# c-zhou/oatk

Measured on AMD Instinct MI355X. Metric: HiFi Gbases/s through syncasm (syncmer+syncerr) at k=1001 s=31, higher is better.
Workload: dtype u64

## Files before the change

oatk_amd/csrc/api.hip:

```cpp
#include <hip/hip_runtime.h>
#include <rocprim/device/device_radix_sort.hpp>
#include <rocprim/device/device_scan.hpp>
#include <rocprim/device/device_transform.hpp>
#include <stdio.h>
#include <stdlib.h>
#include <string.h>
#include <time.h>
#include <execinfo.h>
#include <sys/mman.h>
#include <condition_variable>
#include <mutex>
#include <string>
#include <thread>
#include <utility>
#include <vector>

#include "../../include/oatk_hip.h"
#include "common.hpp"
#include "scan_hpc.hpp"
#include "scan_syncmer.hpp"
#include "scan_syncmer_fast.hpp"
#include "kmer_hash.hpp"
#include "count.hpp"

// ... 734 lines not shown
{
    uint64_t i = (uint64_t) blockIdx.x * blockDim.x + threadIdx.x;
    if (i < n) iota[first + i] = (uint32_t) (first + i);
}

static void scan_reset_downstream(oatk_hip_ctx *ctx)
{
    ctx->scanned = ctx->counted = false;
    ctx->slots_packed = false;
    if (ctx->ec) ctx->ec->done = ctx->ec->marked = ctx->ec->graph_resident = ctx->ec->global = false;
    if (ctx->cons) ctx->cons->done = false;
    if (ctx->ag) ctx->ag->done = false;
    if (ctx->ovl) ctx->ovl->done = false;
    if (ctx->ra) ctx->ra->done = false;
    if (ctx->multi) ctx->multi->merged = ctx->multi->ec_done = false;
}

int oatk_hip_device(oatk_hip_ctx *ctx) { return ctx? ctx->device : -1; }

int oatk_hip_d2d(oatk_hip_ctx *ctx, void *d_dst, const void *d_src, uint64_t bytes)
{
    if (!ctx) return OATK_E_NODEV;
    if (bytes == 0) return OATK_OK;
    CK(hipSetDevice(ctx->device));
    CK(hipMemcpyAsync(d_dst, d_src, bytes, hipMemcpyDeviceToDevice, ctx->stream));
    CK(hipStreamSynchronize(ctx->stream));
    return OATK_OK;
}

int oatk_hip_scan_begin(oatk_hip_ctx *ctx, uint64_t sid0, int k, int s)
{
    if (!ctx) return OATK_E_NODEV;
    CK(hipSetDevice(ctx->device));
    if (!(s > 0 && s < 32 && k > s) || k > oatk_hip_max_k()) { ctx->err = "k/s out of range for the device scan"; return OATK_E_ARG; }
    scan_reset_downstream(ctx);
    ctx->d_seq = nullptr, ctx->d_off = nullptr, ctx->d_len = nullptr;
    ctx->n_reads = 0, ctx->seq_bytes = 0, ctx->sid0 = sid0, ctx->K = k, ctx->S = s;
    ctx->retries = 0, ctx->collisions = 0;
    ctx->n_occ = ctx->tot_nn = ctx->tot_lrl = ctx->n_scm_total = 0;
    ctx->nn_sorted_in_2 = ctx->lrl_sorted_in_2 = false;
    ctx->scanned = true;
    return OATK_OK;
}

#define KEEP(buf, bytes, used)                                                                     \
    do {                                                                                           \
        if (!ctx->buf.grow_keep((bytes), (used), ctx->stream)) {                                   \
            ctx->err = "hipMalloc failed for " #buf " (append)";                                   \
            return OATK_E_NOMEM;                                                                   \
        }                                                                                          \
    } while (0)

static int append_ensure(oatk_hip_ctx *ctx, uint64_t nr, uint64_t sb, uint64_t occ, uint64_t nn, uint64_t lrl)
{
    const uint64_t n0 = ctx->n_reads, b0 = ctx->seq_bytes, o0 = ctx->n_occ;
    KEEP(in_off, (nr + 1) * 8, n0 * 8);
    KEEP(hoco_l, nr * 4 + 4, n0 * 4); KEEP(n_scm, nr * 4 + 4, n0 * 4); KEEP(n_nn, nr * 4 + 4, n0 * 4); KEEP(n_lrl, nr * 4 + 4, n0 * 4);
    KEEP(ho_rl, sb + 64, b0);
    KEEP(hoco_s, sb / 4 + 128 + 16 + ctx->import_reserve, b0 / 4 + 64);
    KEEP(scm_off, (nr + 1) * 8, (n0 + 1) * 8);
    KEEP(pos_hash, occ * 8 + 8, o0 * 8); KEEP(pos_lo, occ * 8 + 8, o0 * 8); KEEP(pos_smer, occ * 8 + 8, o0 * 8); KEEP(pos_mpos, occ * 4 + 4, o0 * 4);
    KEEP(key_hash, occ * 8 + 8, o0 * 8); KEEP(iota, occ * 4 + 4, o0 * 4);
    KEEP(nn_key, nn * 8 + 8, ctx->tot_nn * 8); KEEP(lrl_key, lrl * 8 + 8, ctx->tot_lrl * 8); KEEP(lrl_val, lrl * 4 + 4, ctx->tot_lrl * 4);
    return OATK_OK;
}

int oatk_hip_scan_reserve(oatk_hip_ctx *ctx, uint64_t seq_bytes, uint64_t n_reads, uint64_t n_occ)
{
    if (!ctx) return OATK_E_NODEV;
    CK(hipSetDevice(ctx->device));
    if (!ctx->scanned || ctx->d_seq) { ctx->err = "oatk_hip_scan_reserve: call oatk_hip_scan_begin first"; return OATK_E_STATE; }
    seq_bytes = (seq_bytes + 63) & ~63ULL;
    if (pool_of_current_device()) {
        const uint64_t sb = ctx->seq_bytes + seq_bytes;
        if (!ctx->ho_rl.reserve(sb + 64, ctx->seq_bytes, ctx->stream) || !ctx->hoco_s.reserve(sb / 4 + 128 + 16 + ctx->import_reserve, ctx->seq_bytes / 4 + 64, ctx->stream)) {
            ctx->err = "oatk_hip_scan_reserve: no address range for the batch";
            return OATK_E_NOMEM;
        }
        return OATK_OK;
    }
    return append_ensure(ctx, ctx->n_reads + n_reads, ctx->seq_bytes + seq_bytes, ctx->n_occ + n_occ, ctx->tot_nn, ctx->tot_lrl);
}

int oatk_hip_scan_append(oatk_hip_ctx *ctx, oatk_hip_ctx *src)
{
    if (!ctx || !src) return OATK_E_NODEV;
    CK(hipSetDevice(ctx->device));
    if (ctx == src || ctx->device != src->device) { ctx->err = "oatk_hip_scan_append: the piece must be another handle on the same device"; return OATK_E_ARG; }
    if (!ctx->scanned || ctx->d_seq) { ctx->err = "oatk_hip_scan_append: call oatk_hip_scan_begin first"; return OATK_E_STATE; }
    if (!src->scanned) { ctx->err = "oatk_hip_scan_append: the piece holds no scan"; return OATK_E_STATE; }
    const uint64_t n0 = ctx->n_reads, n1 = src->n_reads, b0 = ctx->seq_bytes, b1 = src->seq_bytes, o0 = ctx->n_occ, o1 = src->n_occ;
    if (n1 == 0) return OATK_OK;
    if (src->K != ctx->K || src->S != ctx->S) { ctx->err = "oatk_hip_scan_append: the piece was scanned with another k / s"; return OATK_E_ARG; }
    if (src->sid0 != ctx->sid0 + n0) { ctx->err = "oatk_hip_scan_append: the piece's first read id must continue the batch"; return OATK_E_ARG; }
    if (n0 + n1 >= 0xFFFFFFFFULL || o0 + o1 > 0xFFFFFFF0ULL) { ctx->err = "oatk_hip_scan_append: batch too large"; return OATK_E_ARG; }
    scan_reset_downstream(ctx);
    ctx->scanned = true;
    { int rc = append_ensure(ctx, n0 + n1, b0 + b1, o0 + o1, ctx->tot_nn + src->tot_nn, ctx->tot_lrl + src->tot_lrl); if (rc) return rc; }
    if (hipStreamSynchronize(src->stream) != hipSuccess) { ctx->err = "oatk_hip_scan_append: the piece's stream failed"; return OATK_E_NODEV; }
    hipStream_t st = ctx->stream;
    auto blocks = [](uint64_t n) { return dim3((unsigned) ((n + 255) / 256 > 0? (n + 255) / 256 : 1)); };
    auto d2d = [&](void *dst, const void *from, size_t bytes) { return bytes? hipMemcpyAsync(dst, from, bytes, hipMemcpyDeviceToDevice, st) : hipSuccess; };
    CK(d2d(ctx->ho_rl.as<uint8_t>() + b0, src->ho_rl.p, b1));
    CK(d2d(ctx->hoco_s.as<uint8_t>() + b0 / 4, src->hoco_s.p, b1 / 4 + 64));
    CK(d2d(ctx->hoco_l.as<uint32_t>() + n0, src->hoco_l.p, n1 * 4)); CK(d2d(ctx->n_scm.as<uint32_t>() + n0, src->n_scm.p, n1 * 4));
    CK(d2d(ctx->n_nn.as<uint32_t>() + n0, src->n_nn.p, n1 * 4)); CK(d2d(ctx->n_lrl.as<uint32_t>() + n0, src->n_lrl.p, n1 * 4));
    hipLaunchKernelGGL(append_rebase_kernel, blocks(n1), dim3(256), 0, st, src->d_off, ctx->in_off.as<uint64_t>() + n0, n1, b0);
    hipLaunchKernelGGL(append_rebase_kernel, blocks(n1 + 1), dim3(256), 0, st, src->scm_off.as<uint64_t>(), ctx->scm_off.as<uint64_t>() + n0, n1 + 1, o0);
    if (o1) {
        CK(d2d(ctx->pos_hash.as<uint64_t>() + o0, src->pos_hash.p, o1 * 8)); CK(d2d(ctx->pos_lo.as<uint64_t>() + o0, src->pos_lo.p, o1 * 8));
        CK(d2d(ctx->pos_smer.as<uint64_t>() + o0, src->pos_smer.p, o1 * 8)); CK(d2d(ctx->pos_mpos.as<uint32_t>() + o0, src->pos_mpos.p, o1 * 4));
        CK(d2d(ctx->key_hash.as<uint64_t>() + o0, src->key_hash.p, o1 * 8));
        hipLaunchKernelGGL(append_iota_kernel, blocks(o1), dim3(256), 0, st, ctx->iota.as<uint32_t>(), o0, o1);
    }
    CK(d2d(ctx->nn_key.as<uint64_t>() + ctx->tot_nn, src->nn_sorted_in_2? src->nn_key2.p : src->nn_key.p, src->tot_nn * 8));
    CK(d2d(ctx->lrl_key.as<uint64_t>() + ctx->tot_lrl, src->lrl_sorted_in_2? src->lrl_key2.p : src->lrl_key.p, src->tot_lrl * 8));
    CK(d2d(ctx->lrl_val.as<uint32_t>() + ctx->tot_lrl, src->lrl_sorted_in_2? src->lrl_val2.p : src->lrl_val.p, src->tot_lrl * 4));
    CK(hipGetLastError());
    CK(hipStreamSynchronize(st));
    ctx->d_off = ctx->in_off.as<uint64_t>();
    ctx->n_reads = n0 + n1, ctx->seq_bytes = b0 + b1, ctx->n_occ = o0 + o1;
    ctx->tot_nn += src->tot_nn, ctx->tot_lrl += src->tot_lrl;
    ctx->retries += src->retries;
    return OATK_OK;
}

int oatk_hip_scan_host(oatk_hip_ctx *ctx, const uint8_t *h_seq, const uint64_t *h_off, const uint32_t *h_len,
                       uint64_t n_reads, uint64_t seq_bytes, uint64_t sid0, int k, int s)
{
    if (!ctx) return OATK_E_NODEV;
    CK(hipSetDevice(ctx->device));
    ENSURE(in_seq, seq_bytes + 64); ENSURE(in_off, (n_reads + 1) * 8); ENSURE(in_len, (n_reads + 1) * 4);
    if (seq_bytes) CK(hipMemcpyAsync(ctx->in_seq.p, h_seq, seq_bytes, hipMemcpyHostToDevice, ctx->stream));
    if (n_reads) {
        CK(hipMemcpyAsync(ctx->in_off.p, h_off, n_reads * 8, hipMemcpyHostToDevice, ctx->stream));
        CK(hipMemcpyAsync(ctx->in_len.p, h_len, n_reads * 4, hipMemcpyHostToDevice, ctx->stream));
    }
    return oatk_hip_scan(ctx, ctx->in_seq.as<uint8_t>(), ctx->in_off.as<uint64_t>(), ctx->in_len.as<uint32_t>(), n_reads, seq_bytes, sid0, k, s);
}

int oatk_hip_count(oatk_hip_ctx *ctx)
{
    using namespace oatk;
    if (!ctx) return OATK_E_NODEV;
    if (!ctx->scanned) { ctx->err = "count before scan"; return OATK_E_STATE; }
    CK(hipSetDevice(ctx->device));
    ctx->counted = false;
    ctx->n_scm_total = 0;
    if (ctx->multi) ctx->multi->merged = ctx->multi->ec_done = false;
    const uint64_t n = ctx->n_occ;
    if (n == 0) { ctx->counted = true; return OATK_OK; }
    const unsigned nb = (unsigned) ((n + 255) / 256);

    ENSURE(key_sorted, n * 8); ENSURE(perm, n * 4); ENSURE(head, n * 4); ENSURE(head_idx, n * 4); ENSURE(newclus, n * 4); ENSURE(kloc, n * 8);
    if (ctx->seq_bytes >> 4 >= 0xFFFFFFFFULL) { ctx->err = "batch too large for 32-bit hoco word indices (64 GB of bases)"; return OATK_E_ARG; }
    ENSURE(clus_id, n * 4); ENSURE(bad_head, n * 4); ENSURE(tag, n * 4); ENSURE(tmp_perm, n * 4); ENSURE(flags, 64);
    ENSURE(pos_kid, n * 8); ENSURE(scm_occ, n * 8);
    CK(hipMemsetAsync(ctx->flags.p, 0, 64, ctx->stream));

    bool full_sort = getenv("OATK_DEBUG_FULL_SORT") != nullptr || n < (1ull << 22);
sort_again:
    t_begin(ctx, OATK_T_COUNT_SORT);
    {
        const unsigned lo_bit = full_sort? 0u : (unsigned) OATK_SORT_LOW_BITS;
        size_t tb = 0;
        CK(rocprim::radix_sort_pairs(nullptr, tb, ctx->key_hash.as<uint64_t>(), ctx->key_sorted.as<uint64_t>(), ctx->iota.as<uint32_t>(),
                                     ctx->perm.as<uint32_t>(), n, lo_bit, 64, ctx->stream));
        ENSURE(tmp, tb);
        CK(rocprim::radix_sort_pairs(ctx->tmp.p, tb, ctx->key_hash.as<uint64_t>(), ctx->key_sorted.as<uint64_t>(), ctx->iota.as<uint32_t>(),
                                     ctx->perm.as<uint32_t>(), n, lo_bit, 64, ctx->stream));
        if (!full_sort) {
            uint32_t *owner = ctx->head.as<uint32_t>();
            CK(hipMemsetAsync(owner, 0xFF, n * 4, ctx->stream));
            hipLaunchKernelGGL(sort_repair_find_kernel, dim3(nb), dim3(256), 0, ctx->stream, ctx->key_sorted.as<uint64_t>(), (uint32_t) n, owner, ctx->flags.as<uint32_t>());
            hipLaunchKernelGGL(sort_repair_kernel, dim3(nb), dim3(256), 0, ctx->stream, ctx->key_sorted.as<uint64_t>(), ctx->perm.as<uint32_t>(), (uint32_t) n, owner,
                               ctx->flags.as<uint32_t>());
        }
    }
    t_end(ctx, OATK_T_COUNT_SORT);

    t_begin(ctx, OATK_T_COUNT_GROUP);
    GroupArgs g;
    g.sorted_key = ctx->key_sorted.as<uint64_t>(), g.perm = ctx->perm.as<uint32_t>(), g.n_rec = (uint32_t) n;
    g.pos_lo = ctx->pos_lo.as<uint64_t>(), g.pos_mpos = ctx->pos_mpos.as<uint32_t>(), g.hoco_s = ctx->hoco_s.as<uint8_t>();
    g.off = ctx->d_off, g.sid0 = ctx->sid0, g.K = ctx->K;
    g.head = ctx->head.as<uint32_t>(), g.head_idx = ctx->head_idx.as<uint32_t>(), g.newclus = ctx->newclus.as<uint32_t>();
    g.loc = ctx->kloc.as<uint64_t>();
    ENSURE(smer_sorted, n * 8);
    g.pos_smer = ctx->pos_smer.as<uint64_t>(), g.occ_sorted = ctx->scm_occ.as<uint64_t>(), g.smer_sorted = ctx->smer_sorted.as<uint64_t>();
    g.flags = ctx->flags.as<uint32_t>();
    ENSURE(slot_rec, n * 32);
    g.slot_rec = ctx->slot_rec.as<uint4>();
    if (!ctx->slots_packed) {
        hipLaunchKernelGGL(pack_slots_kernel, dim3(nb), dim3(256), 0, ctx->stream, g);
        ctx->slots_packed = true;
    }
    hipLaunchKernelGGL((pair_sum_kernel<false>), dim3(2048), dim3(256), 0, ctx->stream, ctx->key_hash.as<uint64_t>(), (const uint32_t *) nullptr, (uint32_t) n, ctx->flags.as<uint32_t>(), 8,
                       (uint32_t *) nullptr, (uint32_t *) nullptr, (uint32_t *) nullptr);
    hipLaunchKernelGGL((pair_sum_kernel<true>), dim3(2048), dim3(256), 0, ctx->stream, ctx->key_sorted.as<uint64_t>(), ctx->perm.as<uint32_t>(), (uint32_t) n, ctx->flags.as<uint32_t>(), 12,
                       g.head, g.newclus, g.head_idx);
    {
        size_t tb = 0;
        CK(rocprim::inclusive_scan(nullptr, tb, ctx->head_idx.as<uint32_t>(), ctx->head_idx.as<uint32_t>(), n, rocprim::maximum<uint32_t>(), ctx->stream));
        ENSURE(tmp, tb);
        CK(rocprim::inclusive_scan(ctx->tmp.p, tb, ctx->head_idx.as<uint32_t>(), ctx->head_idx.as<uint32_t>(), n, rocprim::maximum<uint32_t>(), ctx->stream));
    }
    uint32_t n_scm = 0;
    FinishArgs f;
    auto ids = [&]() -> int {
        size_t tb = 0;
        CK(rocprim::inclusive_scan(nullptr, tb, ctx->newclus.as<uint32_t>(), ctx->clus_id.as<uint32_t>(), n, rocprim::plus<uint32_t>(), ctx->stream));
        ENSURE(tmp, tb);
        CK(rocprim::inclusive_scan(ctx->tmp.p, tb, ctx->newclus.as<uint32_t>(), ctx->clus_id.as<uint32_t>(), n, rocprim::plus<uint32_t>(), ctx->stream));
        uint32_t last_id = 0;
        CK(hipMemcpyAsync(&last_id, ctx->clus_id.as<uint32_t>() + (n - 1), 4, hipMemcpyDeviceToHost, ctx->stream));
        CK(hipStreamSynchronize(ctx->stream));
        n_scm = last_id;
        ENSURE(scm_h, (size_t) n_scm * 8); ENSURE(scm_s, (size_t) n_scm * 8); ENSURE(scm_cov, (size_t) n_scm * 4); ENSURE(scm_loc, (size_t) n_scm * 8);
        ENSURE(scm_occ_off, ((size_t) n_scm + 1) * 8);
        f.perm = ctx->perm.as<uint32_t>(), f.newclus = ctx->newclus.as<uint32_t>(), f.clus_id1 = ctx->clus_id.as<uint32_t>(), f.n_rec = (uint32_t) n;
        f.sorted_key = ctx->key_sorted.as<uint64_t>(), f.smer_sorted = ctx->smer_sorted.as<uint64_t>();
        f.loc = ctx->kloc.as<uint64_t>(), f.scm_loc = ctx->scm_loc.as<uint64_t>();
        f.scm_h = ctx->scm_h.as<uint64_t>(), f.scm_s = ctx->scm_s.as<uint64_t>(), f.scm_occ_off = ctx->scm_occ_off.as<uint64_t>();
        f.scm_occ = ctx->scm_occ.as<uint64_t>(), f.pos_kid = ctx->pos_kid.as<uint64_t>(), f.flags = ctx->flags.as<uint32_t>();
        return OATK_OK;
    };
    { int rc = ids(); if (rc) return rc; }
    hipLaunchKernelGGL(gather_finish_kernel, dim3(nb), dim3(256), 0, ctx->stream, g, f, ctx->clus_id.as<uint32_t>(), n_scm);
    CK(hipMemsetAsync(ctx->bad_head.p, 0, n * 4, ctx->stream));
    hipLaunchKernelGGL(verify_group_kernel, dim3((unsigned) ((n + 8 * OATK_VG_STRIP - 1) / (8 * OATK_VG_STRIP))), dim3(256), 0, ctx->stream, g, ctx->bad_head.as<uint32_t>());
    uint32_t fl[16];
    CK(hipMemcpyAsync(fl, ctx->flags.p, sizeof(fl), hipMemcpyDeviceToHost, ctx->stream));
    CK(hipStreamSynchronize(ctx->stream));
    const bool sort_bad = fl[4] != 0 || memcmp(fl + 8, fl + 12, 16) != 0 || (!full_sort && getenv("OATK_DEBUG_SORT_DISTRUST") != nullptr);
    if (sort_bad && full_sort) {
        t_end(ctx, OATK_T_COUNT_GROUP);
        ctx->err = "the device sort returned something that is not its input in order (rocPRIM radix_sort_pairs): refusing to build the syncmer table from it";
        return OATK_E_NODEV;
    }
    if ((fl[3] || sort_bad) && !full_sort) {
        t_end(ctx, OATK_T_COUNT_GROUP);
        CK(hipMemsetAsync(ctx->flags.p, 0, 64, ctx->stream));
        full_sort = true;
        goto sort_again;
    }
    if (fl[0]) {
        ctx->collisions = 1;
        hipLaunchKernelGGL(split_collisions_kernel, dim3(nb), dim3(256), 0, ctx->stream, g, ctx->bad_head.as<uint32_t>(), ctx->perm.as<uint32_t>(),
                           ctx->tag.as<uint32_t>(), ctx->tmp_perm.as<uint32_t>());
        hipLaunchKernelGGL(regather_kernel, dim3(nb), dim3(256), 0, ctx->stream, g);
        { int rc = ids(); if (rc) return rc; }
        hipLaunchKernelGGL(finish_heads_kernel, dim3(nb), dim3(256), 0, ctx->stream, f, n_scm);
    }
    hipLaunchKernelGGL(check_smer_kernel, dim3(nb), dim3(256), 0, ctx->stream, f);
    hipLaunchKernelGGL(cov_kernel, dim3((n_scm + 255) / 256), dim3(256), 0, ctx->stream, ctx->scm_occ_off.as<uint64_t>(), ctx->scm_cov.as<uint32_t>(), n_scm);
    t_end(ctx, OATK_T_COUNT_GROUP);
    CK(hipGetLastError());
    CK(hipMemcpyAsync(fl, ctx->flags.p, sizeof(fl), hipMemcpyDeviceToHost, ctx->stream));
    CK(hipStreamSynchronize(ctx->stream));
    if (ctx->timing) t_collect(ctx, OATK_T_COUNT_SORT, OATK_T_COUNT_GROUP);
    if (fl[2]) { ctx->err = "hash group with too many distinct k-mers"; return OATK_E_SPLIT; }
    if (debug_refuse(ctx, 4, "oatk_hip_count")) return OATK_E_SPLIT;
    if (fl[1]) { ctx->err = "identical kmers have different smers"; return OATK_E_SMER; }
    ctx->n_scm_total = n_scm;
    ctx->counted = true;
    return OATK_OK;
}

int oatk_hip_info(oatk_hip_ctx *ctx, oatk_hip_info_t *out)
{
    if (!ctx) return OATK_E_NODEV;
    out->n_reads = ctx->n_reads, out->seq_bytes = ctx->seq_bytes, out->sid0 = ctx->sid0;
    out->k = ctx->K, out->s = ctx->S;
    out->n_occ = ctx->n_occ, out->n_nn = ctx->tot_nn, out->n_lrl = ctx->tot_lrl;
    out->n_scm = ctx->n_scm_total;
    out->scan_retries = ctx->retries, out->collisions = ctx->collisions;
    return OATK_OK;
}

int oatk_hip_buffer(oatk_hip_ctx *ctx, int which, const void **d_ptr, uint64_t *bytes)
{
    if (!ctx) return OATK_E_NODEV;
    if (which >= OATK_BUF_INGEST_SEQ && which <= OATK_BUF_INGEST_HDR) return ing_buffer(ctx, which, d_ptr, bytes);
    if (which >= OATK_BUF_MG_H && which <= OATK_BUF_MG_LCOV) return multi_buffer(ctx, which, d_ptr, bytes);
    if (which >= OATK_BUF_MG_G_H && which <= OATK_BUF_MG_POS_GKID) return multi_tail_buffer(ctx, which, d_ptr, bytes);
    if (!ctx->scanned) { ctx->err = "no resident scan"; return OATK_E_STATE; }
    const uint64_t n = ctx->n_reads, occ = ctx->n_occ, ns = ctx->n_scm_total;
    const void *p = nullptr;
    uint64_t b = 0;
    switch (which) {
        case OATK_BUF_HOCO_L: p = ctx->hoco_l.p, b = n * 4; break;
        case OATK_BUF_N_SCM: p = ctx->n_scm.p, b = n * 4; break;
        case OATK_BUF_N_NN: p = ctx->n_nn.p, b = n * 4; break;
        case OATK_BUF_N_LRL: p = ctx->n_lrl.p, b = n * 4; break;
        case OATK_BUF_HO_RL: p = ctx->ho_rl.p, b = ctx->seq_bytes; break;
        case OATK_BUF_HOCO_S: p = ctx->hoco_s.p, b = ctx->seq_bytes / 4 + 64; break;
        case OATK_BUF_NN_KEY: p = ctx->nn_sorted_in_2? ctx->nn_key2.p : ctx->nn_key.p, b = ctx->tot_nn * 8; break;
        case OATK_BUF_LRL_KEY: p = ctx->lrl_sorted_in_2? ctx->lrl_key2.p : ctx->lrl_key.p, b = ctx->tot_lrl * 8; break;
        case OATK_BUF_LRL_VAL: p = ctx->lrl_sorted_in_2? ctx->lrl_val2.p : ctx->lrl_val.p, b = ctx->tot_lrl * 4; break;
        case OATK_BUF_SCM_OFF: p = ctx->scm_off.p, b = (n + 1) * 8; break;
        case OATK_BUF_POS_MPOS: p = ctx->pos_mpos.p, b = occ * 4; break;
        case OATK_BUF_POS_SMER: p = ctx->pos_smer.p, b = occ * 8; break;
        case OATK_BUF_POS_HASH: p = ctx->pos_hash.p, b = occ * 8; break;
        default:
            if (!ctx->counted) { ctx->err = "count results requested before oatk_hip_count"; return OATK_E_STATE; }
            switch (which) {
                case OATK_BUF_POS_KID: p = ctx->pos_kid.p, b = occ * 8; break;
                case OATK_BUF_SCM_H: p = ctx->scm_h.p, b = ns * 8; break;
                case OATK_BUF_SCM_S: p = ctx->scm_s.p, b = ns * 8; break;
                case OATK_BUF_SCM_COV: p = ctx->scm_cov.p, b = ns * 4; break;
                case OATK_BUF_SCM_OCC_OFF: p = ctx->scm_occ_off.p, b = (ns + 1) * 8; break;
                case OATK_BUF_SCM_OCC: p = ctx->scm_occ.p, b = occ * 8; break;
                default:
                    if (which >= OATK_BUF_CONS_SEL && which <= OATK_BUF_CONS_TOT) return cons_buffer(ctx, which, d_ptr, bytes);
                    if (which >= OATK_BUF_AG_SCM_DEL && which <= OATK_BUF_AG_ARC_LINK) return ag_buffer(ctx, which, d_ptr, bytes);
                    if (which >= OATK_BUF_OVL_KEY && which <= OATK_BUF_OVL_TAIL) return ovl_buffer(ctx, which, d_ptr, bytes);
                    if (which >= OATK_BUF_RA_ALN_SID && which <= OATK_BUF_RA_SKIPPED) return ra_buffer(ctx, which, d_ptr, bytes);
                    if (which >= OATK_BUF_INGEST_SEQ && which <= OATK_BUF_INGEST_HDR) return ing_buffer(ctx, which, d_ptr, bytes);
                    return ec_buffer(ctx, which, d_ptr, bytes);
            }
    }
    *d_ptr = p, *bytes = b;
    return OATK_OK;
}

void *oatk_hip_staging(oatk_hip_ctx *ctx, uint64_t bytes)
{
    if (!ctx || hipSetDevice(ctx->device) != hipSuccess) return nullptr;
    if (bytes <= ctx->staging_cap) return ctx->staging;
    staging_free(ctx);
    const uint64_t HP = 2ull << 20, want = (bytes + HP - 1) & ~(HP - 1);
    void *raw = mmap(nullptr, want + HP, PROT_READ | PROT_WRITE, MAP_PRIVATE | MAP_ANONYMOUS, -1, 0);
    if (raw != MAP_FAILED) {
        uint8_t *base = (uint8_t *) (((uintptr_t) raw + HP - 1) & ~(uintptr_t) (HP - 1));
        (void) madvise(base, want, MADV_HUGEPAGE);
        const int nt = want >= (256ull << 20)? 8 : 1;
        std::vector<std::thread> th;
        for (int t = 1; t < nt; ++t) th.emplace_back([=] { for (uint64_t o = want / nt * t; o < (t + 1 == nt? want : want / nt * (t + 1)); o += 4096) *(volatile uint8_t *) (base + o) = 0; });
        for (uint64_t o = 0; o < want / nt; o += 4096) *(volatile uint8_t *) (base + o) = 0;
        for (auto &x : th) x.join();
        if (hipHostRegister(base, want, hipHostRegisterDefault) == hipSuccess) {
            ctx->staging = base, ctx->staging_cap = want, ctx->staging_raw = raw, ctx->staging_raw_size = want + HP;
            return ctx->staging;
        }
        (void) hipGetLastError();
        munmap(raw, want + HP);
    }
    if (hipHostMalloc(&ctx->staging, bytes, hipHostMallocDefault) != hipSuccess) { ctx->staging = nullptr; ctx->err = "hipHostMalloc failed (staging)"; return nullptr; }
    ctx->staging_cap = bytes;
    return ctx->staging;
}

int oatk_hip_host_register(oatk_hip_ctx *ctx, void *p, uint64_t bytes)
{
    if (!ctx) return OATK_E_NODEV;
    if (!p || bytes == 0) return OATK_E_ARG;
    CK(hipSetDevice(ctx->device));
    CK(hipHostRegister(p, bytes, hipHostRegisterDefault));
    return OATK_OK;
}

int oatk_hip_host_unregister(oatk_hip_ctx *ctx, void *p)
{
    if (!ctx) return OATK_E_NODEV;
    CK(hipSetDevice(ctx->device));
    CK(hipHostUnregister(p));
    return OATK_OK;
}

int oatk_hip_d2h(oatk_hip_ctx *ctx, void *h_dst, const void *d_src, uint64_t bytes)
{
    if (!ctx) return OATK_E_NODEV;
    if (bytes == 0) return OATK_OK;
    CK(hipSetDevice(ctx->device));
    CK(hipMemcpyAsync(h_dst, d_src, bytes, hipMemcpyDeviceToHost, ctx->stream));
    CK(hipStreamSynchronize(ctx->stream));
    return OATK_OK;
}

int oatk_hip_d2h_async(oatk_hip_ctx *ctx, void *h_dst, const void *d_src, uint64_t bytes)
{
    if (!ctx) return OATK_E_NODEV;
    if (bytes == 0) return OATK_OK;
// ... 16 lines not shown
```

oatk_amd/csrc/count.hpp:

```cpp
#pragma once
#include "common.hpp"

namespace oatk {

__device__ __forceinline__ uint64_t kmer_word_global(const uint32_t *hs32, uint32_t pos, uint32_t rev, int K, int wd)
{
    int32_t t = rev? (int32_t) pos + K - 32 - 32 * wd : (int32_t) pos + 32 * wd;
    int nb = K - 32 * wd;
    nb = nb > 32? 32 : nb;
    int32_t wi = t >> 4;
    uint32_t sh = ((uint32_t) t & 15u) * 2u;
    uint32_t w0, w1, w2;
    if (wi >= 0) {
        struct __attribute__((packed, aligned(4))) W3 { uint32_t a, b, c; };
        const W3 v = *(const W3 *) (hs32 + wi);
        w0 = __builtin_bswap32(v.a), w1 = __builtin_bswap32(v.b), w2 = __builtin_bswap32(v.c);
    } else {
        w0 = 0u;
        w1 = wi + 1 >= 0? __builtin_bswap32(hs32[wi + 1]) : 0u;
        w2 = wi + 2 >= 0? __builtin_bswap32(hs32[wi + 2]) : 0u;
    }
    uint64_t hi = (uint64_t) w0 << 32 | w1;
    uint64_t V = sh? (hi << sh) | ((uint64_t) w2 >> (32u - sh)) : hi;
    if (rev) V = revcomp32(V);
    if (nb < 32) V &= ~0ULL << (64 - 2 * nb);
    return V;
}

struct GroupArgs {
    const uint64_t *sorted_key;
    const uint32_t *perm;
    uint32_t n_rec;
    const uint64_t *pos_lo;
    const uint32_t *pos_mpos;
    const uint8_t *hoco_s;
    const uint64_t *off;
    uint64_t sid0;
    int K;
    uint32_t *head;
    uint32_t *head_idx;
    uint32_t *newclus;
    uint32_t *flags;
    uint64_t *loc;
    const uint64_t *pos_smer;
    uint64_t *occ_sorted, *smer_sorted;
    uint4 *slot_rec;
};

__global__ void pack_slots_kernel(GroupArgs a)
{
    uint32_t p = blockIdx.x * blockDim.x + threadIdx.x;
    if (p >= a.n_rec) return;
    const uint64_t lo = a.pos_lo[p], sm = a.pos_smer[p];
    const uint64_t loc = ((a.off[(lo >> 32) - a.sid0] >> 4) << 32) | a.pos_mpos[p];
    a.slot_rec[2 * (size_t) p] = make_uint4((uint32_t) lo, (uint32_t) (lo >> 32), (uint32_t) sm, (uint32_t) (sm >> 32));
    a.slot_rec[2 * (size_t) p + 1] = make_uint4((uint32_t) loc, (uint32_t) (loc >> 32), 0u, 0u);
}

#define OATK_SORT_LOW_BITS 24
#define OATK_SORT_REPAIR_MAX 4096u
__device__ __forceinline__ bool sort_repair_boundary(const uint64_t *key, uint32_t n, uint32_t i, uint32_t &start, uint32_t *flags)
{
    if (i == 0 || i >= n) return false;
    const uint64_t k = key[i], kp = key[i - 1];
    if ((k >> OATK_SORT_LOW_BITS) != (kp >> OATK_SORT_LOW_BITS) || k == kp) return false;
    uint32_t s = i - 1;
    while (s > 0 && (key[s - 1] >> OATK_SORT_LOW_BITS) == (k >> OATK_SORT_LOW_BITS)) {
        --s;
        if (i - s > OATK_SORT_REPAIR_MAX) { flags[3] = 1u; return false; }
    }
    start = s;
    return true;
}
__global__ void sort_repair_find_kernel(const uint64_t *key, uint32_t n, uint32_t *owner, uint32_t *flags)
{
    const uint32_t i = blockIdx.x * blockDim.x + threadIdx.x;
    uint32_t s;
    if (sort_repair_boundary(key, n, i, s, flags)) atomicMin(&owner[s], i);
    if (i > 0 && i < n && (key[i] >> OATK_SORT_LOW_BITS) < (key[i - 1] >> OATK_SORT_LOW_BITS)) flags[3] = 1u;
}
__global__ void sort_repair_kernel(uint64_t *key, uint32_t *perm, uint32_t n, uint32_t *owner, uint32_t *flags)
{
    const uint32_t i = blockIdx.x * blockDim.x + threadIdx.x;
    uint32_t s;
    if (!sort_repair_boundary(key, n, i, s, flags) || owner[s] != i) return;
    const uint64_t top = key[i] >> OATK_SORT_LOW_BITS;
    uint32_t e = i + 1;
    while (e < n && (key[e] >> OATK_SORT_LOW_BITS) == top) {
        ++e;
        if (e - s > OATK_SORT_REPAIR_MAX) { flags[3] = 1u; return; }
    }
    for (uint32_t a = i; a < e; ++a) {
        const uint64_t kk = key[a];
        const uint32_t pp = perm[a];
        uint32_t b = a;
        while (b > s && key[b - 1] > kk) { key[b] = key[b - 1], perm[b] = perm[b - 1]; --b; }
        key[b] = kk, perm[b] = pp;
    }
}

__device__ __forceinline__ void pair_sums(uint64_t key, uint32_t slot, uint64_t &s0, uint64_t &s1)
{
    uint64_t x = key ^ ((uint64_t) slot * 0x9E3779B97F4A7C15ULL);
    x ^= x >> 32; x *= 0xD6E8FEB86659FD93ULL; x ^= x >> 32;
    s0 = x;
    x *= 0xD6E8FEB86659FD93ULL; x ^= x >> 29; x += key;
    s1 = x;
}
template <bool HEADS>
__global__ __launch_bounds__(256) void pair_sum_kernel(const uint64_t *key, const uint32_t *perm, uint32_t n, uint32_t *flags, int at,
                                                       uint32_t *head, uint32_t *newclus, uint32_t *head_idx)
{
    __shared__ uint64_t part[2][4];
    uint64_t s0 = 0, s1 = 0;
    bool inv = false;
    const uint64_t stride = (uint64_t) gridDim.x * blockDim.x;
    for (uint64_t i0 = (uint64_t) blockIdx.x * blockDim.x + threadIdx.x; i0 < n; i0 += 4 * stride) {
        uint64_t k[4], kp[4];
        uint32_t v[4];
#pragma unroll
        for (int u = 0; u < 4; ++u) {
            const uint64_t i = i0 + u * stride;
            const bool in = i < n;
            k[u] = in? key[i] : 0, v[u] = in? (perm? perm[i] : (uint32_t) i) : 0, kp[u] = in && perm && i? key[i - 1] : 0;
        }
#pragma unroll
        for (int u = 0; u < 4; ++u) {
            if (i0 + u * stride >= n) continue;
            uint64_t a, b;
            pair_sums(k[u], v[u], a, b);
            s0 += a, s1 += b;
            if (k[u] < kp[u]) inv = true;
            if (HEADS) {
                const uint32_t i = (uint32_t) (i0 + u * stride), h = i == 0 || k[u] != kp[u];
                head[i] = h, newclus[i] = h, head_idx[i] = h? i : 0u;
            }
        }
    }
    #pragma unroll
    for (int d = 32; d > 0; d >>= 1) s0 += __shfl_xor(s0, d), s1 += __shfl_xor(s1, d);
    if ((threadIdx.x & 63u) == 0) part[0][threadIdx.x >> 6] = s0, part[1][threadIdx.x >> 6] = s1;
    if (inv) flags[4] = 1u;
    __syncthreads();
    if (threadIdx.x == 0) {
        atomicAdd((unsigned long long *) (flags + at), (unsigned long long) (part[0][0] + part[0][1] + part[0][2] + part[0][3]));
        atomicAdd((unsigned long long *) (flags + at + 2), (unsigned long long) (part[1][0] + part[1][1] + part[1][2] + part[1][3]));
    }
}

__global__ void mark_heads_kernel(GroupArgs a)
{
    uint32_t i = blockIdx.x * blockDim.x + threadIdx.x;
    if (i >= a.n_rec) return;
    uint32_t h = i == 0 || a.sorted_key[i] != a.sorted_key[i - 1];
    a.head[i] = h;
    a.newclus[i] = h;
    a.head_idx[i] = h? i : 0u;
    const uint32_t p = a.perm[i];
    const uint4 r0 = a.slot_rec[2 * (size_t) p], r1 = a.slot_rec[2 * (size_t) p + 1];
    a.loc[i] = (uint64_t) r1.y << 32 | r1.x;
    a.occ_sorted[i] = (uint64_t) r0.y << 32 | r0.x, a.smer_sorted[i] = (uint64_t) r0.w << 32 | r0.z;
}
__global__ void regather_kernel(GroupArgs a)
{
    uint32_t i = blockIdx.x * blockDim.x + threadIdx.x;
    if (i >= a.n_rec) return;
    const uint32_t p = a.perm[i];
    const uint4 r0 = a.slot_rec[2 * (size_t) p], r1 = a.slot_rec[2 * (size_t) p + 1];
    a.loc[i] = (uint64_t) r1.y << 32 | r1.x;
    a.occ_sorted[i] = (uint64_t) r0.y << 32 | r0.x, a.smer_sorted[i] = (uint64_t) r0.w << 32 | r0.z;
}

#ifndef OATK_VG_STRIP
#define OATK_VG_STRIP 8
#endif
#ifndef OATK_VFY_WAVES
#define OATK_VFY_WAVES 1
#endif
__global__ __launch_bounds__(256, OATK_VFY_WAVES) void verify_group_kernel(GroupArgs a, uint32_t *bad_head)
{
    const uint32_t hl = threadIdx.x & 31, half0 = threadIdx.x & 32;
    const uint32_t i0 = (uint32_t) OATK_VG_STRIP * (blockIdx.x * (blockDim.x >> 5) + (threadIdx.x >> 5));
    uint32_t my_h = 0;
    uint64_t my_lp = 0, my_lq = 0;
    bool my_live = false;
    if (hl < OATK_VG_STRIP) {
        const uint32_t i = i0 + hl;
        my_live = i < a.n_rec && !a.head[i];
        if (my_live) {
            my_h = a.head_idx[i];
            my_lp = a.loc[i];
            my_lq = a.loc[my_h];
        }
    }
    const uint64_t live_mask = (__ballot(my_live) >> half0) & ((1ULL << OATK_VG_STRIP) - 1ULL);
    if (live_mask == 0) return;
    const uint32_t *hs32 = (const uint32_t *) a.hoco_s;
    const int nw = (a.K + 31) / 32;
    uint32_t diff = 0;
    const uint32_t first_live = (uint32_t) __builtin_ctzll(live_mask);
    const uint64_t lq0 = (uint64_t) __shfl((long long) my_lq, (int) (half0 + first_live));
    const bool one_head = __ballot(my_live && my_lq != lq0) == 0;
    for (int w0 = 0; w0 < nw; w0 += 32) {
        const int wd = w0 + (int) hl;
        const bool in = wd < nw;
        uint64_t p[OATK_VG_STRIP], q[OATK_VG_STRIP];
        if (one_head) {
            const uint64_t q0 = in? kmer_word_global(hs32 + (lq0 >> 32), (uint32_t) lq0 >> 1, (uint32_t) lq0 & 1u, a.K, wd) : 0;
#pragma unroll
            for (int r = 0; r < OATK_VG_STRIP; ++r) {
                const uint64_t lp = (uint64_t) __shfl((long long) my_lp, (int) (half0 + r));
                const bool live = in && ((live_mask >> r) & 1u);
                p[r] = live? kmer_word_global(hs32 + (lp >> 32), (uint32_t) lp >> 1, (uint32_t) lp & 1u, a.K, wd) : q0;
            }
#pragma unroll
            for (int r = 0; r < OATK_VG_STRIP; ++r) diff |= (uint32_t) (p[r] != q0) << r;
        } else {
#pragma unroll
            for (int r = 0; r < OATK_VG_STRIP; ++r) {
                const uint64_t lp = (uint64_t) __shfl((long long) my_lp, (int) (half0 + r)), lq = (uint64_t) __shfl((long long) my_lq, (int) (half0 + r));
                const bool live = in && ((live_mask >> r) & 1u);
                p[r] = live? kmer_word_global(hs32 + (lp >> 32), (uint32_t) lp >> 1, (uint32_t) lp & 1u, a.K, wd) : 0;
                q[r] = live? kmer_word_global(hs32 + (lq >> 32), (uint32_t) lq >> 1, (uint32_t) lq & 1u, a.K, wd) : 0;
            }
#pragma unroll
            for (int r = 0; r < OATK_VG_STRIP; ++r) diff |= (uint32_t) (p[r] != q[r]) << r;
        }
    }
#pragma unroll
    for (int r = 0; r < OATK_VG_STRIP; ++r) {
        const uint64_t bad = (__ballot((diff >> r) & 1u) >> half0) & 0xFFFFFFFFULL;
        if (bad && hl == (uint32_t) r) a.flags[0] = 1u, bad_head[my_h] = 1u;
    }
}

#define OATK_MAX_SPLIT 16
__global__ void split_collisions_kernel(GroupArgs a, const uint32_t *bad_head, uint32_t *perm_rw, uint32_t *tag, uint32_t *tmp_perm)
{
    uint32_t i = blockIdx.x * blockDim.x + threadIdx.x;
    if (i >= a.n_rec || !a.head[i] || !bad_head[i]) return;
    uint32_t e = i + 1;
    while (e < a.n_rec && !a.head[e]) ++e;
    const int nw = (a.K + 31) / 32;
    uint32_t rep[OATK_MAX_SPLIT], nclus = 0;
    for (uint32_t t = i; t < e; ++t) {
        uint32_t p = perm_rw[t];
        uint64_t lo_p = a.pos_lo[p];
        const uint32_t *hs_p = (const uint32_t *) (a.hoco_s + (a.off[(lo_p >> 32) - a.sid0] >> 2));
        uint32_t mp = a.pos_mpos[p], c;
        for (c = 0; c < nclus; ++c) {
            uint32_t q = perm_rw[rep[c]];
            uint64_t lo_q = a.pos_lo[q];
            const uint32_t *hs_q = (const uint32_t *) (a.hoco_s + (a.off[(lo_q >> 32) - a.sid0] >> 2));
            uint32_t mq = a.pos_mpos[q];
            bool same = true;
            for (int wd = 0; wd < nw && same; ++wd)
                same = kmer_word_global(hs_p, mp >> 1, mp & 1u, a.K, wd) == kmer_word_global(hs_q, mq >> 1, mq & 1u, a.K, wd);
            if (same) break;
        }
        if (c == nclus) {
            if (nclus == OATK_MAX_SPLIT) { a.flags[2] = 1u; return; }
            rep[nclus++] = t;
        }
        tag[t] = c;
    }
    uint32_t w = i;
    for (uint32_t c = 0; c < nclus; ++c) {
        bool first = true;
        for (uint32_t t = i; t < e; ++t)
            if (tag[t] == c) {
                tmp_perm[w] = perm_rw[t];
                a.newclus[w] = first? 1u : 0u;
                first = false;
                ++w;
            }
    }
    for (uint32_t t = i; t < e; ++t) perm_rw[t] = tmp_perm[t];
}

struct FinishArgs {
    const uint32_t *perm;
    const uint32_t *newclus;
    const uint32_t *clus_id1;
    uint32_t n_rec;
    const uint64_t *sorted_key, *smer_sorted;
    uint64_t *scm_h, *scm_s;
    uint64_t *scm_occ_off;
    uint64_t *scm_occ;
    const uint64_t *loc;
    uint64_t *scm_loc;
    uint64_t *pos_kid;
    uint32_t *flags;
};

__global__ void finish_heads_kernel(FinishArgs a, uint32_t n_scm)
{
    uint32_t i = blockIdx.x * blockDim.x + threadIdx.x;
    if (i >= a.n_rec) return;
    uint32_t p = a.perm[i], id = a.clus_id1[i] - 1u;
    a.pos_kid[p] = (uint64_t) id << 1;
    if (a.newclus[i]) {
        a.scm_h[id] = a.sorted_key[i];
        a.scm_s[id] = a.smer_sorted[i];
        a.scm_occ_off[id] = i;
        a.scm_loc[id] = a.loc[i];
    }
    if (i == a.n_rec - 1) a.scm_occ_off[n_scm] = a.n_rec;
}

__global__ void gather_finish_kernel(GroupArgs g, FinishArgs a, const uint32_t *clus_id1, uint32_t n_scm)
{
    uint32_t i = blockIdx.x * blockDim.x + threadIdx.x;
    if (i >= a.n_rec) return;
    const uint32_t p = g.perm[i], id = clus_id1[i] - 1u;
    const uint4 r0 = g.slot_rec[2 * (size_t) p], r1 = g.slot_rec[2 * (size_t) p + 1];
    const uint64_t loc = (uint64_t) r1.y << 32 | r1.x, smer = (uint64_t) r0.w << 32 | r0.z;
    g.loc[i] = loc;
    g.occ_sorted[i] = (uint64_t) r0.y << 32 | r0.x, g.smer_sorted[i] = smer;
    a.pos_kid[p] = (uint64_t) id << 1;
    if (g.newclus[i]) {
        a.scm_h[id] = a.sorted_key[i];
        a.scm_s[id] = smer;
        a.scm_occ_off[id] = i;
        a.scm_loc[id] = loc;
    }
    if (i == a.n_rec - 1) a.scm_occ_off[n_scm] = a.n_rec;
}

__global__ void check_smer_kernel(FinishArgs a)
{
    uint32_t i = blockIdx.x * blockDim.x + threadIdx.x;
    if (i >= a.n_rec) return;
    uint32_t id = a.clus_id1[i] - 1u;
    if (a.smer_sorted[i] != a.scm_s[id]) a.flags[1] = 1u;
}

__global__ void cov_kernel(const uint64_t *occ_off, uint32_t *cov, uint32_t n_scm)
{
    uint32_t i = blockIdx.x * blockDim.x + threadIdx.x;
    if (i < n_scm) cov[i] = (uint32_t) (occ_off[i + 1] - occ_off[i]);
}

}
```

Measured before the change: 374.9.

## Verify k-mer groups against cluster representative slots, skip head_idx scan

By default the count stage no longer builds head_idx or runs the max inclusive scan that propagated group heads. A new verify_slots_kernel compares each occurrence's k-mer against its cluster's representative location (scm_loc) read via pos_kid. It stages the block's contiguous span of packed sequence words into shared memory, byte-swapped, and falls back to global fetches when the span is too large. The old verify_group path stays behind an environment flag; the change adds risk around the correctness of the new comparison indexing.

```diff
diff --git a/oatk_amd/csrc/api.hip b/oatk_amd/csrc/api.hip
--- a/oatk_amd/csrc/api.hip
+++ b/oatk_amd/csrc/api.hip
@@ -910,7 +910,10 @@
     if (n == 0) { ctx->counted = true; return OATK_OK; }
     const unsigned nb = (unsigned) ((n + 255) / 256);
 
-    ENSURE(key_sorted, n * 8); ENSURE(perm, n * 4); ENSURE(head, n * 4); ENSURE(head_idx, n * 4); ENSURE(newclus, n * 4); ENSURE(kloc, n * 8);
+    bool verify_sorted;
+    { const char *e = getenv("OATK_DEBUG_COUNT_VERIFY_SORTED"); verify_sorted = e && e[0] == '1'; }
+    ENSURE(key_sorted, n * 8); ENSURE(perm, n * 4); ENSURE(head, n * 4); ENSURE(newclus, n * 4); ENSURE(kloc, n * 8);
+    if (verify_sorted) ENSURE(head_idx, n * 4);
     if (ctx->seq_bytes >> 4 >= 0xFFFFFFFFULL) { ctx->err = "batch too large for 32-bit hoco word indices (64 GB of bases)"; return OATK_E_ARG; }
     ENSURE(clus_id, n * 4); ENSURE(bad_head, n * 4); ENSURE(tag, n * 4); ENSURE(tmp_perm, n * 4); ENSURE(flags, 64);
     ENSURE(pos_kid, n * 8); ENSURE(scm_occ, n * 8);
@@ -942,7 +945,7 @@
     g.sorted_key = ctx->key_sorted.as<uint64_t>(), g.perm = ctx->perm.as<uint32_t>(), g.n_rec = (uint32_t) n;
     g.pos_lo = ctx->pos_lo.as<uint64_t>(), g.pos_mpos = ctx->pos_mpos.as<uint32_t>(), g.hoco_s = ctx->hoco_s.as<uint8_t>();
     g.off = ctx->d_off, g.sid0 = ctx->sid0, g.K = ctx->K;
-    g.head = ctx->head.as<uint32_t>(), g.head_idx = ctx->head_idx.as<uint32_t>(), g.newclus = ctx->newclus.as<uint32_t>();
+    g.head = ctx->head.as<uint32_t>(), g.head_idx = verify_sorted? ctx->head_idx.as<uint32_t>() : nullptr, g.newclus = ctx->newclus.as<uint32_t>();
     g.loc = ctx->kloc.as<uint64_t>();
     ENSURE(smer_sorted, n * 8);
     g.pos_smer = ctx->pos_smer.as<uint64_t>(), g.occ_sorted = ctx->scm_occ.as<uint64_t>(), g.smer_sorted = ctx->smer_sorted.as<uint64_t>();
@@ -957,7 +960,7 @@
                        (uint32_t *) nullptr, (uint32_t *) nullptr, (uint32_t *) nullptr);
     hipLaunchKernelGGL((pair_sum_kernel<true>), dim3(2048), dim3(256), 0, ctx->stream, ctx->key_sorted.as<uint64_t>(), ctx->perm.as<uint32_t>(), (uint32_t) n, ctx->flags.as<uint32_t>(), 12,
                        g.head, g.newclus, g.head_idx);
-    {
+    if (verify_sorted) {
         size_t tb = 0;
         CK(rocprim::inclusive_scan(nullptr, tb, ctx->head_idx.as<uint32_t>(), ctx->head_idx.as<uint32_t>(), n, rocprim::maximum<uint32_t>(), ctx->stream));
         ENSURE(tmp, tb);
@@ -986,7 +989,16 @@
     { int rc = ids(); if (rc) return rc; }
     hipLaunchKernelGGL(gather_finish_kernel, dim3(nb), dim3(256), 0, ctx->stream, g, f, ctx->clus_id.as<uint32_t>(), n_scm);
     CK(hipMemsetAsync(ctx->bad_head.p, 0, n * 4, ctx->stream));
-    hipLaunchKernelGGL(verify_group_kernel, dim3((unsigned) ((n + 8 * OATK_VG_STRIP - 1) / (8 * OATK_VG_STRIP))), dim3(256), 0, ctx->stream, g, ctx->bad_head.as<uint32_t>());
+    {
+        const dim3 vgrid((unsigned) ((n + 8 * OATK_VG_STRIP - 1) / (8 * OATK_VG_STRIP)));
+        if (verify_sorted) hipLaunchKernelGGL(verify_group_kernel, vgrid, dim3(256), 0, ctx->stream, g, ctx->bad_head.as<uint32_t>());
+        else {
+            SlotVerifyArgs sv;
+            sv.pos_kid = ctx->pos_kid.as<uint64_t>(), sv.scm_loc = ctx->scm_loc.as<uint64_t>(), sv.scm_occ_off = ctx->scm_occ_off.as<uint64_t>();
+            sv.n_scm = n_scm, sv.span_max = (uint32_t) OATK_VS_SPAN;
+            hipLaunchKernelGGL(verify_slots_kernel, vgrid, dim3(256), 0, ctx->stream, g, sv, ctx->bad_head.as<uint32_t>());
+        }
+    }
     uint32_t fl[16];
     CK(hipMemcpyAsync(fl, ctx->flags.p, sizeof(fl), hipMemcpyDeviceToHost, ctx->stream));
     CK(hipStreamSynchronize(ctx->stream));
diff --git a/oatk_amd/csrc/count.hpp b/oatk_amd/csrc/count.hpp
--- a/oatk_amd/csrc/count.hpp
+++ b/oatk_amd/csrc/count.hpp
@@ -133,7 +133,8 @@
             if (k[u] < kp[u]) inv = true;
             if (HEADS) {
                 const uint32_t i = (uint32_t) (i0 + u * stride), h = i == 0 || k[u] != kp[u];
-                head[i] = h, newclus[i] = h, head_idx[i] = h? i : 0u;
+                head[i] = h, newclus[i] = h;
+                if (head_idx) head_idx[i] = h? i : 0u;
             }
         }
     }
@@ -231,6 +232,133 @@
     for (int r = 0; r < OATK_VG_STRIP; ++r) {
         const uint64_t bad = (__ballot((diff >> r) & 1u) >> half0) & 0xFFFFFFFFULL;
         if (bad && hl == (uint32_t) r) a.flags[0] = 1u, bad_head[my_h] = 1u;
+    }
+}
+
+#ifndef OATK_VS_SPAN
+#define OATK_VS_SPAN 4096
+#endif
+struct SlotVerifyArgs {
+    const uint64_t *pos_kid;
+    const uint64_t *scm_loc;
+    const uint64_t *scm_occ_off;
+    uint32_t n_scm;
+    uint32_t span_max;
+};
+struct KmerW3 { uint32_t a, b, c; };
+__device__ __forceinline__ KmerW3 kmer_fetch3(const uint32_t *hs32, uint64_t loc, int K, int wd, bool use, uint32_t idle, uint32_t &meta)
+{
+    const uint32_t pos = (uint32_t) loc >> 1, rev = (uint32_t) loc & 1u;
+    const int32_t t = rev? (int32_t) pos + K - 32 - 32 * wd : (int32_t) pos + 32 * wd;
+    const int64_t w = (int64_t) (loc >> 32) + (t >> 4);
+    const uint32_t miss = w < 0? (uint32_t) -w : 0u;
+    meta = (((uint32_t) t & 15u) * 2u) | rev << 8 | miss << 9;
+    struct __attribute__((packed, aligned(4))) W3 { uint32_t a, b, c; };
+    const W3 v = *(const W3 *) (hs32 + (!use? idle : miss? 0u : (uint32_t) w));
+    return KmerW3{v.a, v.b, v.c};
+}
+template <bool SWAPPED>
+__device__ __forceinline__ uint64_t kmer_finish3(KmerW3 v, uint32_t meta)
+{
+    uint32_t w0 = SWAPPED? v.a : __builtin_bswap32(v.a), w1 = SWAPPED? v.b : __builtin_bswap32(v.b), w2 = SWAPPED? v.c : __builtin_bswap32(v.c);
+    const uint32_t miss = meta >> 9, sh = meta & 63u;
+    if (miss) {
+        w2 = miss == 1? w1 : miss == 2? w0 : 0u;
+        w1 = miss == 1? w0 : 0u;
+        w0 = 0u;
+    }
+    const uint32_t hi = (uint32_t) ((((uint64_t) w0 << 32 | w1) << sh) >> 32), lo = (uint32_t) ((((uint64_t) w1 << 32 | w2) << sh) >> 32);
+    const uint64_t V = (uint64_t) hi << 32 | lo;
+    return (meta >> 8) & 1u? revcomp32(V) : V;
+}
+__global__ __launch_bounds__(256) void verify_slots_kernel(GroupArgs a, SlotVerifyArgs s, uint32_t *bad_head)
+{
+    __shared__ uint32_t span[OATK_VS_SPAN];
+    __shared__ uint32_t span_lo, span_hi;
+    const uint32_t hl = threadIdx.x & 31, half0 = threadIdx.x & 32;
+    const uint64_t p0 = (uint64_t) OATK_VG_STRIP * ((uint64_t) blockIdx.x * (blockDim.x >> 5) + (threadIdx.x >> 5));
+    const uint32_t *hs32 = (const uint32_t *) a.hoco_s;
+    const int nw = (a.K + 31) / 32;
+    if (threadIdx.x == 0) span_lo = 0xFFFFFFFFu, span_hi = 0u;
+    __syncthreads();
+    uint32_t my_id = 0;
+    uint64_t my_lp = 0, my_lq = 0;
+    bool my_live = false;
+    if (hl < OATK_VG_STRIP) {
+        const uint64_t p = p0 + hl;
+        if (p < a.n_rec) {
+            my_lp = ((const uint64_t *) a.slot_rec)[4 * p + 2];
+            my_id = (uint32_t) (s.pos_kid[p] >> 1);
+            if (my_id < s.n_scm) {
+                my_lq = s.scm_loc[my_id];
+                my_live = my_lq != my_lp;
+                my_lq ^= my_lp & 1u;
+            }
+        }
+        if (my_live) {
+            const uint32_t pos = (uint32_t) my_lp >> 1, rw = (uint32_t) (my_lp >> 32);
+            atomicMin(&span_lo, rw + (pos >> 4));
+            atomicMax(&span_hi, rw + ((pos + (uint32_t) a.K - 1u) >> 4) + 3u);
+        }
+    }
+    __syncthreads();
+    const uint32_t lo = span_lo & ~3u, hi = span_hi;
+    const bool staged = hi > lo && hi - lo <= s.span_max;
+    if (staged) {
+        const uint32_t n4 = (hi - lo) >> 2;
+        for (uint32_t w = threadIdx.x; w < n4; w += blockDim.x) {
+            const uint4 v = ((const uint4 *) (hs32 + lo))[w];
+            span[4 * w] = __builtin_bswap32(v.x), span[4 * w + 1] = __builtin_bswap32(v.y), span[4 * w + 2] = __builtin_bswap32(v.z), span[4 * w + 3] = __builtin_bswap32(v.w);
+        }
+        if (threadIdx.x < ((hi - lo) & 3u)) span[4 * n4 + threadIdx.x] = __builtin_bswap32(hs32[lo + 4 * n4 + threadIdx.x]);
+    }
+    __syncthreads();
+    const uint64_t live_mask = (__ballot(my_live) >> half0) & ((1ULL << OATK_VG_STRIP) - 1ULL);
+    if (live_mask == 0) return;
+    uint32_t diff = 0;
+    const uint32_t my_pw = !my_live? 0u : (((uint32_t) (my_lp >> 32) - lo + (((uint32_t) my_lp >> 1) >> 4)) << 8) | ((((uint32_t) my_lp >> 1) & 15u) * 2u);
+    const uint64_t my_lpf = my_lp & ~1ULL;
+    for (int w0 = 0; w0 < nw; w0 += 32) {
+        const bool in = w0 + (int) hl < nw;
+        const int wd = in? w0 + (int) hl : 0;
+        const int nb = a.K - 32 * wd;
+        const uint64_t wmask = !in? 0ULL : nb < 32? ~0ULL << (64 - 2 * nb) : ~0ULL;
+        KmerW3 p[OATK_VG_STRIP], q[OATK_VG_STRIP];
+        uint32_t pm[OATK_VG_STRIP], qm[OATK_VG_STRIP];
+#pragma unroll
+        for (int r = 0; r < OATK_VG_STRIP; ++r) {
+            const uint64_t lq = (uint64_t) __shfl((long long) my_lq, (int) (half0 + r));
+            q[r] = kmer_fetch3(hs32, lq, a.K, wd, (live_mask >> r) & 1u, lo, qm[r]);
+        }
+        if (staged) {
+#pragma unroll
+            for (int r = 0; r < OATK_VG_STRIP; ++r) {
+                const uint32_t pw = (uint32_t) __shfl((int) my_pw, (int) (half0 + r));
+                const uint32_t *w = span + (pw >> 8) + 2 * wd;
+                p[r] = KmerW3{w[0], w[1], w[2]}, pm[r] = pw & 0xFFu;
+            }
+        } else {
+#pragma unroll
+            for (int r = 0; r < OATK_VG_STRIP; ++r) {
+                const uint64_t lp = (uint64_t) __shfl((long long) my_lpf, (int) (half0 + r));
+                p[r] = kmer_fetch3(hs32, lp, a.K, wd, (live_mask >> r) & 1u, lo, pm[r]);
+            }
+        }
+#pragma unroll
+        for (int r = 0; r < OATK_VG_STRIP; ++r) {
+            const uint64_t P = staged? kmer_finish3<true>(p[r], pm[r]) : kmer_finish3<false>(p[r], pm[r]), Q = kmer_finish3<false>(q[r], qm[r]);
+            diff |= (uint32_t) (((P ^ Q) & wmask) != 0) << r;
+        }
+    }
+    diff &= (uint32_t) live_mask;
+#pragma unroll
+    for (int r = 0; r < OATK_VG_STRIP; ++r) {
+        const uint64_t bad = (__ballot((diff >> r) & 1u) >> half0) & 0xFFFFFFFFULL;
+        if (bad && hl == (uint32_t) r) {
+            const uint64_t h = s.scm_occ_off[my_id];
+            a.flags[0] = 1u;
+            if (h < a.n_rec) bad_head[h] = 1u;
+        }
     }
 }
 
```

Result: slower. 368.9 (-1.6%).
